# ChaoqinRobotics/LINS---LiDAR-inertial-SLAM

Hardware: NVIDIA H100
Metric: ESKF iterations/sec (higher is better)
Workload: dtype f64 (f32 association)

## Files before the change

lins---lidar-inertial-slam_b200/csrc/cuda/lins_assoc.cuh:

```cuda
#pragma once
#include "lins_assoc_az.cuh"

namespace lins_dev {

constexpr int kGroupLanes = 4;
constexpr int kThreadScanBins = 16, kThreadWalkBins = 48;

constexpr int kCertSlots = 40, kPassSlots = 48;
__device__ __forceinline__ void count_cert_events(long long* timers, unsigned ev) {
#pragma unroll
  for (int k = 0; k < 8; ++k) {
    const unsigned n1 = __popc(__ballot_sync(0xffffffffu, (ev >> k) & 1u)), n2 = __popc(__ballot_sync(0xffffffffu, (ev >> (8 + k)) & 1u));
    if ((threadIdx.x & 31) == 0 && (n1 | n2)) atomicAdd((unsigned long long*)&timers[kCertSlots + k], ((unsigned long long)n2 << 32) | n1);
  }
}

struct PassBuffers {
  float4* qpt;
  float4* sel;
  unsigned long long* key;
  int* pos;
  float4* qa;
  int4* qw;
  float4* qref;
// ... 88 lines not shown
    float4 qa = make_float4(0.f, 0.f, -1.f, 0.f);
    if (seeded) {
      const float4 r1 = pb.qref[v], r2 = pb.qref2[v], ex = pb.qext[v];
      const unsigned nearbits = __float_as_uint(nearf);
      const int w1s = pb.pos[3 * v], w2s = pb.pos[3 * v + 1], w3s = pb.pos[3 * v + 2];
      const int r1s = __float_as_int(ex.y), r2s = __float_as_int(ex.z), r3s = __float_as_int(ex.w);
      const int ccr0 = pb.qccr[v];
      const bool walks = ccr0 >= 0;
      auto entry = [&](int slot, bool use) -> float4 {
        return use && slot >= 0 && slot < ixq.T ? ixq.pts[slot] : make_float4(0.f, 0.f, 0.f, 0.f);
      };
      const float4 tw1 = entry(w1s, true), tr1 = entry(r1s, w1s >= 0);
      const float4 tw2 = entry(w2s, walks), tr2 = entry(r2s, walks && w2s >= 0);
      const float4 tw3 = entry(w3s, walks && surf), tr3 = entry(r3s, walks && surf && w3s >= 0);
      const float moved1 = sqrtf(sqdist_f32(s.x, s.y, s.z, r1.x, r1.y, r1.z));
      const int c1 = w1s >= 0 ? cert_check<false>(tw1, tr1, s, r1s, r1.w, moved1, nearbits, 0)
                              : (cert_rejected(r1.w, moved1) ? kCertKeep : kCertFailSlack);
      const bool ok1 = c1 <= kCertSwap;
      ev = 1u | (1u << (ok1 ? 1 : c1)) | (c1 == kCertSwap ? 1u << 7 : 0u);
      if (c1 == kCertSwap) { az_polar(s, qa); pb.qa[v] = qa; pb.qw[v] = make_int4(-4, 0, 0, 0); continue; }
      bool ok2 = false;
      int c2 = kCertKeep, c3 = kCertKeep;
      if (ok1 && walks) {
        const int c0 = ccr0 & 0x00ffffff;
        const float moved2 = sqrtf(sqdist_f32(s.x, s.y, s.z, r2.x, r2.y, r2.z));
        c2 = w2s >= 0 ? cert_check<true>(tw2, tr2, s, r2s, r2.w, moved2, nearbits, c0) : (cert_rejected(r2.w, moved2) ? kCertKeep : kCertFailSlack);
        ok2 = c2 <= kCertSwap;
        if (ok2 && surf) {
          c3 = w3s >= 0 ? cert_check<true>(tw3, tr3, s, r3s, ex.x, moved2, nearbits, c0) : (cert_rejected(ex.x, moved2) ? kCertKeep : kCertFailSlack);
          ok2 = c3 <= kCertSwap;
        }
        ev |= (1u << 8) | (1u << (8 + (ok2 ? 1 : c2 <= kCertSwap ? c3 : c2))) |
              (ok2 && (c2 == kCertSwap || c3 == kCertSwap) ? 1u << 15 : 0u);
      }
      if (ok1 && (ok2 || ccr0 < 0)) { pb.qw[v] = make_int4(-2, (c2 == kCertSwap ? 1 : 0) | (c3 == kCertSwap ? 2 : 0), 0, 0); continue; }
      if (ok1) { az_polar(s, qa); pb.qa[v] = qa; pb.qw[v] = make_int4(-3, 0, 0, 0); continue; }
    }
    const int w1 = az_prepare_nn(ixq, s, nearf, seeded ? pb.pos[3 * v] : -1, (int)pb.qpt[v].w, qa);
    pb.qa[v] = qa;
    pb.qw[v] = make_int4(w1, 0, 0, 0);
    if (sm.first_pass && w1 >= 0 && (w1 & 0xffff) <= kThreadScanBins) pb.wl[NQ - 1 - atomicAdd(&cta.wl_tn[0], 1)] = v;
    else pb.wl[atomicAdd(&cta.wl_n[0], 1)] = v;
    if (bv.timers && w1 >= 0) atomicAdd(&cta.dbg[0], w1 & 0xffff);
    } while (false);
    if (bv.timers) count_cert_events(bv.timers, ev);
  }
  __syncthreads();
  LINS_TICK_PASS(3);

  if (cta.any_indexed) {
    if (bv.timers && threadIdx.x == 0) {
      atomicAdd((unsigned long long*)&bv.timers[10], (unsigned long long)cta.wl_n[0]);
      atomicAdd((unsigned long long*)&bv.timers[12], (unsigned long long)cta.dbg[0]);
    }
    const float gate = sqrtf(nearf);
    auto nn_finish = [&](int v, const AzIndex& ix, const float4 s, const Top3& top, int w1, float Bout) {
      const unsigned long long k1 = top.k1;
      const int p1 = top.p1;
      const float d1 = __uint_as_float((unsigned)(k1 >> 32));
      const bool acc1 = k1 != kKeyMax && p1 >= 0 && (double)d1 < kp.nearest_sq;
      if (bv.timers && !slots[slot_of(v, Q)].first_pass && pb.pos[3 * v] >= 0 && acc1 && (p1 == pb.pos[3 * v] || p1 == __float_as_int(pb.qext[v].y)))
        atomicAdd((unsigned long long*)&bv.timers[kCertSlots + 6], 1ull);
      const float bound1 = w1 < 0 ? -1.f : acc1 ? cert_bound(top.d3, Bout) : rejected_slack((unsigned)(k1 >> 32), Bout, gate);
      pb.qref[v] = make_float4(s.x, s.y, s.z, bound1);
      pb.qext[v].y = __int_as_float(acc1 ? top.p2 : -1);
      pb.pos[3 * v] = acc1 ? p1 : -1;
      pb.qccr[v] = acc1 ? ((slot_ring(ix.pts[p1].w) << 24) | (int)(unsigned)(k1 & 0xffffffffu)) : -1;
    };
    constexpr int G = kGroupLanes;
    const int sub = lane & (G - 1), glead = lane & ~(G - 1);
    const unsigned gmask = G == 32 ? 0xffffffffu : (((1u << G) - 1u) << glead);
    for (;;) {
      int k = 0;
      if (sub == 0) k = atomicAdd(&cta.wl_thead[0], 1);
      k = __shfl_sync(gmask, k, glead);
      if (k >= cta.wl_tn[0]) break;
      const int v = pb.wl[NQ - 1 - k];
      const int sl = slot_of(v, Q), i = v - sl * Q;
      const Smem& sm = slots[sl];
      const AzIndex ix = az_index_of(sm, bv, i < sm.ns);
      const float4 s = pb.sel[v];
      const int w1 = pb.qw[v].x;
      const float4 qag = pb.qa[v];
      const Top3 top = az_scan_nn_group<G>(ix, s, w1, qag.y, qag.w, sub, gmask);
      if (sub == 0) nn_finish(v, ix, s, top, w1, qag.w);
    }
    for (;;) {
      int k = 0;
      if (lane == 0) k = atomicAdd(&cta.wl_head[0], 1);
      k = __shfl_sync(0xffffffffu, k, 0);
      if (k >= cta.wl_n[0]) break;
      const int v = pb.wl[k];
      const int sl = slot_of(v, Q), i = v - sl * Q;
      const Smem& sm = slots[sl];
      int w1 = pb.qw[v].x;
      Top3 top;
      top.init();
      const bool surf = i < sm.ns;
      const AzIndex ix = az_index_of(sm, bv, surf);
      const float4 s = pb.sel[v];
      float4 qa = pb.qa[v];
      if (w1 >= 0) {
        const int wp = sm.first_pass ? az_probe_window(ix, qa, w1) : -1;
        if (wp >= 0) {
          const Top3 pr = az_scan_nn(ix, s, wp, qa.y, sqrtf(widen(kProbeSq)));
          if (pr.p1 >= 0) {
            w1 = az_nn_window(ix, az_seed_bound(ix, s, pr.p1, nearf), qa);
            if (lane == 0) pb.qa[v] = qa;
          }
        }
        top = az_scan_nn(ix, s, w1, qa.y, qa.w);
      }
      if (lane == 0) nn_finish(v, ix, s, top, w1, qa.w);
    }
    __syncthreads();
    if (bv.timers && threadIdx.x == 0 && !cta.pass_first) {
      const int n = cta.wl_n[0] + cta.wl_tn[0], b = n == 0 ? 0 : n <= 16 ? 1 : 2;
      atomicAdd((unsigned long long*)&bv.timers[kPassSlots + b], 1ull);
      atomicAdd((unsigned long long*)&bv.timers[kPassSlots + 3 + b], (unsigned long long)(clock64() - cta.tlast));
    }
    LINS_TICK_PASS(4);
    for (int v = threadIdx.x; v < NQ; v += kThreads) {
      const int sl = slot_of(v, Q), i = v - sl * Q;
      const Smem& sm = slots[sl];
      if (!sm.run || !sm.az_ok || i >= sm.ns + sm.nc || (sm.iter % kp.icp_freq) != 0) continue;
      const int2 lq = *reinterpret_cast<const int2*>(&pb.qw[v]);
      const int lvl = lq.x;
      const bool surf = i < sm.ns;
      auto swap_front = [&](int k, float* runner_up) {
        const int w = pb.pos[3 * v + k], r = __float_as_int(*runner_up);
        pb.pos[3 * v + k] = r;
        *runner_up = __int_as_float(w);
        return az_index_of(sm, bv, surf).pts[r].w;
      };
      if (lvl == -2) {
        if (lq.y) {
          int* const o = surf ? bv.ind_s + 3 * (size_t)(sm.qs0 + i) : bv.ind_c + 2 * (size_t)(sm.qc0 + i - sm.ns);
          if (lq.y & 1) o[1] = slot_index(swap_front(1, &pb.qext[v].z));
          if (lq.y & 2) o[2] = slot_index(swap_front(2, &pb.qext[v].w));
        }
        continue;
      }
      if (lvl == -4) {
        const float tw = swap_front(0, &pb.qext[v].y);
        pb.qccr[v] = (slot_ring(tw) << 24) | slot_index(tw);
      }
      const int ccr = pb.qccr[v];
      if (ccr < 0) {
        pb.pos[3 * v + 1] = -1; pb.pos[3 * v + 2] = -1;
        pb.qw[v] = make_int4(-1, 0, 0, 0);
        if (surf) { int* o = bv.ind_s + 3 * (size_t)(sm.qs0 + i); o[0] = -1; o[1] = -1; o[2] = -1; }
        else { int* o = bv.ind_c + 2 * (size_t)(sm.qc0 + i - sm.ns); o[0] = -1; o[1] = -1; }
        continue;
      }
      int w2 = 0, w3 = 0;
      float B2 = 0.f, B3 = 0.f;
      const bool seeded = !sm.first_pass;
      const int sd2 = seeded ? pb.pos[3 * v + 1] : -1, sd3 = seeded ? pb.pos[3 * v + 2] : -1;
      const int c = ccr & 0x00ffffff, cr = (int)((unsigned)ccr >> 24);
      const AzIndex ix = az_index_of(sm, bv, surf);
      const int p1 = pb.pos[3 * v];
      if (surf) az_prepare_walk<true>(ix, pb.sel[v], pb.qa[v], p1, c, cr, sd2, sd3, min(sm.ns, sm.Ts), nearf, w2, w3, B2, B3);
      else az_prepare_walk<false>(ix, pb.sel[v], pb.qa[v], p1, c, cr, sd2, sd3, min(sm.nc, sm.Tc), nearf, w2, w3, B2, B3);
      pb.qw[v] = make_int4(lvl == -3 ? 2 : 1, w2, w3, ccr);
      reinterpret_cast<float2*>(pb.key)[v] = make_float2(B2, B3);
      if (sm.first_pass && (w2 & 0xffff) <= kThreadWalkBins && (w3 & 0xffff) <= kThreadWalkBins) pb.wl[NQ - 1 - atomicAdd(&cta.wl_tn[1], 1)] = v;
      else pb.wl[atomicAdd(&cta.wl_n[1], 1)] = v;
      if (bv.timers) atomicAdd(&cta.dbg[1], (w2 & 0xffff) + 4 * (w3 & 0xffff));
    }
    __syncthreads();
    if (bv.timers && threadIdx.x == 0) {
      atomicAdd((unsigned long long*)&bv.timers[11], (unsigned long long)cta.wl_n[1]);
      atomicAdd((unsigned long long*)&bv.timers[13], (unsigned long long)cta.dbg[1]);
    }
    auto walk_finish = [&](int v, const Smem& sm, int i, bool surf, const float4 s, int ccr, const WalkOut& wo) {
      float4 ex = pb.qext[v];
      if (bv.timers && pb.qw[v].x == 2) {
        auto held = [](int w, int r, int now) { return w >= 0 ? now == w || now == r : now < 0; };
        if (held(pb.pos[3 * v + 1], __float_as_int(ex.z), wo.pos2) && (!surf || held(pb.pos[3 * v + 2], __float_as_int(ex.w), wo.pos3)))
          atomicAdd((unsigned long long*)&bv.timers[kCertSlots + 6], 1ull << 32);
      }
      pb.pos[3 * v + 1] = wo.pos2; pb.pos[3 * v + 2] = wo.pos3;
      pb.qref2[v] = make_float4(s.x, s.y, s.z, wo.bound2);
      ex.x = wo.bound3; ex.z = __int_as_float(wo.run2); ex.w = __int_as_float(wo.run3);
      pb.qext[v] = ex;
      const int i1 = ccr & 0x00ffffff;
      if (surf) { int* o = bv.ind_s + 3 * (size_t)(sm.qs0 + i); o[0] = i1; o[1] = wo.i2; o[2] = wo.i3; }
      else { int* o = bv.ind_c + 2 * (size_t)(sm.qc0 + i - sm.ns); o[0] = i1; o[1] = wo.i2; }
    };
    for (;;) {
      int k = 0;
      if (sub == 0) k = atomicAdd(&cta.wl_thead[1], 1);
      k = __shfl_sync(gmask, k, glead);
      if (k >= cta.wl_tn[1]) break;
      const int v = pb.wl[NQ - 1 - k];
      const int sl = slot_of(v, Q), i = v - sl * Q;
      const Smem& sm = slots[sl];
      const int4 w = pb.qw[v];
      const bool surf = i < sm.ns;
      const float2 B = reinterpret_cast<const float2*>(pb.key)[v];
      const float4 s = pb.sel[v];
      const AzIndex ix = az_index_of(sm, bv, surf);
      const WalkOut wo = surf ? az_scan_walk_group<true, G>(ix, s, w.w, w.y, w.z, min(sm.ns, sm.Ts), nearf, B.x, B.y, sub, gmask)
                              : az_scan_walk_group<false, G>(ix, s, w.w, w.y, w.z, min(sm.nc, sm.Tc), nearf, B.x, B.y, sub, gmask);
      if (sub == 0) walk_finish(v, sm, i, surf, s, w.w, wo);
    }
    for (;;) {
      int k = 0;
      if (lane == 0) k = atomicAdd(&cta.wl_head[1], 1);
      k = __shfl_sync(0xffffffffu, k, 0);
      if (k >= cta.wl_n[1]) break;
      const int v = pb.wl[k];
      const int sl = slot_of(v, Q), i = v - sl * Q;
      const Smem& sm = slots[sl];
      const int4 w = pb.qw[v];
      const bool surf = i < sm.ns;
      const float2 B = reinterpret_cast<const float2*>(pb.key)[v];
      const int w2 = w.y, w3 = w.z;
      const float4 s = pb.sel[v];
      const AzIndex ix = az_index_of(sm, bv, surf);
      const WalkOut wo = surf ? az_scan_walk<true>(ix, s, w.w, w2, w3, min(sm.ns, sm.Ts), nearf, B.x, B.y)
                              : az_scan_walk<false>(ix, s, w.w, w2, w3, min(sm.nc, sm.Tc), nearf, B.x, B.y);
      if (lane == 0) walk_finish(v, sm, i, surf, s, w.w, wo);
    }
  }
  if (cta.any_legacy) {
    for (int sl = 0; sl < bv.nslots; ++sl) {
      const Smem& sm = slots[sl];
      if (!sm.run || sm.az_ok || (sm.iter % kp.icp_freq) != 0) continue;
      const bool sep = nn_separate(bv, sm.scan);
      const float4* __restrict__ nnS = sep ? bv.nn_s + bv.nn_s_off[sm.scan] : bv.ts + sm.ts0;
      const float4* __restrict__ nnC = sep ? bv.nn_c + bv.nn_c_off[sm.scan] : bv.tc + sm.tc0;
      const int TnS = sep ? bv.nn_s_off[sm.scan + 1] - bv.nn_s_off[sm.scan] : sm.Ts;
      const int TnC = sep ? bv.nn_c_off[sm.scan + 1] - bv.nn_c_off[sm.scan] : sm.Tc;
      if (sm.ns > 0 && TnS > 0) nn_brute(pb.sel + sl * Q, pb.key + sl * Q, sm.ns, nnS, TnS);
      if (sm.nc > 0 && TnC > 0) nn_brute(pb.sel + sl * Q + sm.ns, pb.key + sl * Q + sm.ns, sm.nc, nnC, TnC);
    }
    __syncthreads();
    for (int sl = 0; sl < bv.nslots; ++sl) {
      const Smem& sm = slots[sl];
      if (!sm.run || sm.az_ok || (sm.iter % kp.icp_freq) != 0) continue;
      const float4* __restrict__ tgtS = bv.ts + sm.ts0;
      const float4* __restrict__ tgtC = bv.tc + sm.tc0;
      const int fwdS = min(sm.ns, sm.Ts), fwdC = min(sm.nc, sm.Tc);
      for (int i = threadIdx.x; i < sm.ns + sm.nc; i += kThreads) {
        const int v = sl * Q + i;
        const bool surf = i < sm.ns;
        const unsigned long long k1 = pb.key[v];
        const float d1 = __uint_as_float((unsigned)(k1 >> 32));
        const int c = (int)(unsigned)(k1 & 0xffffffffu);
        const bool found = (k1 != kKeyMax) && ((double)d1 < kp.nearest_sq) && c < (surf ? sm.Ts : sm.Tc);
        int i1 = -1, i2 = -1, i3 = -1;
        if (found) {
          i1 = c;
          const float4 s = pb.sel[v];
          if (surf) walk_seq<true>(s, c, tgtS, sm.Ts, fwdS, nearf, i2, i3);
          else walk_seq<false>(s, c, tgtC, sm.Tc, fwdC, nearf, i2, i3);
        }
        pb.pos[3 * v] = i1; pb.pos[3 * v + 1] = i2; pb.pos[3 * v + 2] = i3;
        if (surf) { int* o = bv.ind_s + 3 * (size_t)(sm.qs0 + i); o[0] = i1; o[1] = i2; o[2] = i3; }
        else { int* o = bv.ind_c + 2 * (size_t)(sm.qc0 + i - sm.ns); o[0] = i1; o[1] = i2; }
      }
    }
  }
  __syncthreads();
  if (bv.timers && threadIdx.x == 0 && !cta.pass_first) {
    const int n = cta.wl_n[1] + cta.wl_tn[1], b = n == 0 ? 0 : n <= 16 ? 1 : n <= 32 ? 2 : 3;
    atomicAdd((unsigned long long*)&bv.timers[kPassSlots + 6 + b], 1ull);
    atomicAdd((unsigned long long*)&bv.timers[kPassSlots + 10 + b], (unsigned long long)(clock64() - cta.tlast));
  }
  LINS_TICK_PASS(5);
  if (threadIdx.x == kThreads - 1) { cta.wl_n[0] = 0; cta.wl_n[1] = 0; cta.wl_tn[0] = 0; cta.wl_tn[1] = 0; cta.wl_head[0] = 0; cta.wl_head[1] = 0; cta.wl_thead[0] = 0; cta.wl_thead[1] = 0; cta.dbg[0] = 0; cta.dbg[1] = 0; }

  double* const fold_stage = cta.u.fold[warp];
  for (int v0 = warp * 32; v0 < NQ; v0 += kThreads) {
    const int sl = slot_of(v0, Q), i0 = v0 - sl * Q;
    const Smem& sm = slots[sl];
    const int ntot = sm.ns + sm.nc;
    if (!sm.run || i0 >= ntot) continue;
    const int v = v0 + lane, i = i0 + lane;
    const bool valid = i < ntot;
    const bool surf = i < sm.ns;
    const bool search = (sm.iter % kp.icp_freq) == 0;
    const bool weighted = sm.iter >= kp.icp_freq;
    const bool by_slot = search ? (sm.az_ok != 0) : (sm.pos_valid && sm.pos_is_slot);
    float4 coeff = make_float4(0.f, 0.f, 0.f, 0.f);
    float4 s = make_float4(0.f, 0.f, 0.f, 0.f);
    bool ok = false;
    if (valid) {
      const int i1 = pb.pos[3 * v], i2 = pb.pos[3 * v + 1], i3 = pb.pos[3 * v + 2];
      s = pb.sel[v];
      if (surf) {
        if (i2 >= 0 && i3 >= 0 && i1 >= 0 && i1 < sm.Ts && i2 < sm.Ts && i3 < sm.Ts) {
          const float4* t = by_slot ? bv.az_s + sm.ts0 : bv.ts + sm.ts0;
          ok = plane_residual(s, t[i1], t[i2], t[i3], weighted, coeff);
        }
      } else {
        if (i2 >= 0 && i1 >= 0 && i1 < sm.Tc && i2 < sm.Tc) {
          const float4* t = by_slot ? bv.az_c + sm.tc0 : bv.tc + sm.tc0;
          ok = line_residual(s, t[i1], t[i2], weighted, coeff);
        }
      }
    }
    double g[6] = {0.0, 0.0, 0.0, 0.0, 0.0, 0.0}, r = 0.0;
    if (ok) {
// ... 28 lines not shown
```

lins---lidar-inertial-slam_b200/csrc/cuda/lins_assoc_az.cuh:

```cuda
#pragma once
#include "lins_kernels.cuh"

namespace lins_dev {

struct AzIndex {
  const float4* pts;
  const aztab_t* bstart;
  const int (*elev)[2];
  int nb, nrings, T;
};
__device__ __forceinline__ int float_key(float f) { const int i = __float_as_int(f); return i >= 0 ? i : i ^ 0x7fffffff; }
__device__ __forceinline__ float key_float(int k) { return __int_as_float(k >= 0 ? k : k ^ 0x7fffffff); }
__device__ __forceinline__ float slope_of(float x, float y, float z) {
  return __fdiv_rn(z, sqrtf(__fadd_rn(__fmul_rn(x, x), __fmul_rn(y, y))));
}
__device__ __forceinline__ float ring_lower_bound(const AzIndex& ix, int r, float zq, float rq) {
  const float lo = key_float(ix.elev[r][0]), hi = key_float(ix.elev[r][1]);
  const float a = __fmaf_rn(lo, rq, -zq), b = __fmaf_rn(-hi, rq, zq);
  const float m = a > b ? lo : hi;
  const float bound = fmaxf(a, b) * rsqrtf(__fmaf_rn(m, m, 1.f)) * 0.998f - 1.0e-4f;
  return hi - lo < 1.0e30f ? bound : -1.f;
}

__device__ __forceinline__ int az_bin(float x, float y, int nb) {
  const float a = atan2f(y, x);
  int b = (int)floorf((a + kPiF) * ((float)nb * (0.5f / kPiF)));
  return min(max(b, 0), nb - 1);
}
__device__ __forceinline__ int az_bins_for(int nrings, int tab) {
  int p2 = 1;
  while (p2 < nrings) p2 <<= 1;
  return tab / p2;
}

__device__ __forceinline__ int cnt16_add1(unsigned* cnt, int b) {
  const int sh = (b & 1) * 16;
  return (int)((atomicAdd(&cnt[b >> 1], 1u << sh) >> sh) & 0xffffu);
}
template <int TAB>
__device__ void az_build(const float4* __restrict__ src, int T, float4* dst, aztab_t* table, unsigned* cnt, int* scan_tmp, int nb, int (*elev)[2]) {
  unsigned short* cnt16 = reinterpret_cast<unsigned short*>(cnt);
  for (int w = threadIdx.x; w <= TAB / 2; w += kThreads) cnt[w] = 0u;
  for (int r = threadIdx.x; r < kMaxRing; r += kThreads) { elev[r][0] = float_key(3.0e38f); elev[r][1] = float_key(-3.0e38f); }
  __syncthreads();
  for (int j = threadIdx.x; j < T; j += kThreads) {
    const float4 t = __ldg(&src[j]);
    cnt16_add1(cnt, (int)t.w * nb + az_bin(t.x, t.y, nb));
    const float e = slope_of(t.x, t.y, t.z);
    if (fabsf(e) < 1.0e30f) { const int k = float_key(e); atomicMin(&elev[(int)t.w][0], k); atomicMax(&elev[(int)t.w][1], k); }
    else { atomicMin(&elev[(int)t.w][0], float_key(-3.0e38f)); atomicMax(&elev[(int)t.w][1], float_key(3.0e38f)); }
  }
  __syncthreads();
  constexpr int PER = TAB / kThreads;
  static_assert(PER >= 1 && PER * kThreads == TAB, "table size must be a multiple of the block size");
  int loc[PER];
  int sum = 0;
#pragma unroll
  for (int k = 0; k < PER; ++k) { loc[k] = cnt16[threadIdx.x * PER + k]; sum += loc[k]; }
  scan_tmp[threadIdx.x] = sum;
  __syncthreads();
  if (threadIdx.x < 32) {
    constexpr int PW = kThreads / 32;
    int part[PW];
    int s = 0;
#pragma unroll
    for (int k = 0; k < PW; ++k) { part[k] = scan_tmp[threadIdx.x * PW + k]; s += part[k]; }
    int incl = s;
#pragma unroll
    for (int m = 1; m < 32; m <<= 1) { const int o = __shfl_up_sync(0xffffffffu, incl, m); if ((int)threadIdx.x >= m) incl += o; }
    int run = incl - s;
#pragma unroll
    for (int k = 0; k < PW; ++k) { const int v = part[k]; scan_tmp[threadIdx.x * PW + k] = run; run += v; }
    if (threadIdx.x == 31) table[TAB] = (aztab_t)incl;
  }
  __syncthreads();
  {
    int run = scan_tmp[threadIdx.x];
#pragma unroll
    for (int k = 0; k < PER; ++k) { cnt16[threadIdx.x * PER + k] = (unsigned short)run; table[threadIdx.x * PER + k] = (aztab_t)run; run += loc[k]; }
  }
  __syncthreads();
  for (int j = threadIdx.x; j < T; j += kThreads) {
    const float4 t = __ldg(&src[j]);
    const int pos = cnt16_add1(cnt, (int)t.w * nb + az_bin(t.x, t.y, nb));
    dst[pos] = make_float4(t.x, t.y, t.z, __int_as_float(((int)t.w << 24) | j));
  }
  __syncthreads();
}

__device__ __forceinline__ float az_halfwidth(float U, float rho) {
  const float r = sqrtf(U) * 1.002f + 1.0e-5f;
  if (!(r < rho)) return 4.0f;
  return asinf(r / rho) + 1.0e-5f;
}
__device__ __forceinline__ void az_window(int nb, float aq, float th, int& blo, int& nbins) {
  const float inv_binw = (float)nb * (0.5f / kPiF);
  nbins = (int)(2.0f * th * inv_binw) + 3;
  if (!(th < kPiF) || nbins >= nb) { blo = 0; nbins = nb; return; }
  int b = (int)floorf((aq - th + kPiF) * inv_binw) - 1;
  b %= nb;
  if (b < 0) b += nb;
  blo = b;
}

__device__ __forceinline__ int slot_index(float w) { return __float_as_int(w) & 0x00ffffff; }
__device__ __forceinline__ int slot_ring(float w) { return (int)((unsigned)__float_as_int(w) >> 24); }
__device__ __forceinline__ int pack_window(int blo, int nbins) { return (blo << 16) | nbins; }
constexpr float kCertMargin = 0.1f;
__device__ __forceinline__ float widen(float U) { const float r = sqrtf(U) + kCertMargin; return r * r; }
__device__ __forceinline__ float rejected_slack(unsigned best_bits, float Bout, float gate) {
  const float db = best_bits >= 0x7f800000u ? Bout : fminf(sqrtf(__uint_as_float(best_bits)), Bout);
  return db - gate * 1.00001f;
}

__device__ __forceinline__ void az_polar(const float4 s, float4& qa) {
  qa.x = atan2f(s.y, s.x);
  qa.y = sqrtf(__fadd_rn(__fmul_rn(s.x, s.x), __fmul_rn(s.y, s.y)));
}
__device__ __forceinline__ int az_nn_window(const AzIndex& ix, float U1, float4& qa) {
  const float Uw = widen(U1);
  int blo, nbins;
  az_window(ix.nb, qa.x, az_halfwidth(Uw, qa.y), blo, nbins);
  qa.w = nbins >= ix.nb ? 3.0e38f : sqrtf(Uw);
  return pack_window(blo, nbins);
}
__device__ __forceinline__ float az_seed_bound(const AzIndex& ix, const float4 s, int seed_slot, float U1) {
  if (seed_slot >= 0 && seed_slot < ix.T) {
    const float4 t = ix.pts[seed_slot];
    const float d = sqdist_f32(s.x, s.y, s.z, t.x, t.y, t.z);
    if (d < U1) U1 = d;
  }
  return U1;
}
__device__ __forceinline__ int az_bin_of_angle(float a, int nb) {
  const int b = (int)floorf((a + kPiF) * ((float)nb * (0.5f / kPiF)));
  return min(max(b, 0), nb - 1);
}
__device__ __forceinline__ float az_bucket_bound(const AzIndex& ix, const float4 s, float az, int ring_guess, float U1) {
  const int bq = az_bin_of_angle(az, ix.nb);
  const int r0 = min(max(ring_guess, 0), ix.nrings - 1);
#pragma unroll 1
  for (int k = 0; k < 3; ++k) {
    const int r = k == 0 ? r0 : (k == 1 ? r0 - 1 : r0 + 1);
    if (k == 1 && U1 < 1.0f) break;
    if (r < 0 || r >= ix.nrings) continue;
    const int base = r * ix.nb;
    int p = ix.bstart[base + max(bq - 1, 0)];
    const int pe = min((int)ix.bstart[base + min(bq + 2, ix.nb)], p + 4);
    for (; p < pe; ++p) U1 = az_seed_bound(ix, s, p, U1);
  }
  return U1;
}
__device__ __forceinline__ int az_prepare_nn(const AzIndex& ix, const float4 s, float nearf, int seed_slot, int ring_guess, float4& qa) {
  qa = make_float4(0.f, 0.f, -1.f, 0.f);
  if (!(s.x == s.x && s.y == s.y && s.z == s.z) || ix.T <= 0) return -1;
  az_polar(s, qa);
  float U1 = az_seed_bound(ix, s, seed_slot, nearf);
  if (seed_slot < 0) U1 = az_bucket_bound(ix, s, qa.x, ring_guess, U1);
  return az_nn_window(ix, U1, qa);
}
constexpr float kProbeSq = 0.25f;
__device__ __forceinline__ int az_probe_window(const AzIndex& ix, const float4 qa, int full_window) {
  int blo, nbins;
  az_window(ix.nb, qa.x, az_halfwidth(kProbeSq, qa.y), blo, nbins);
  return (full_window & 0xffff) > 2 * nbins + 4 ? pack_window(blo, nbins) : -1;
}

struct Top3 {
  unsigned long long k1, k2;
  int p1, p2;
  unsigned d3;
  __device__ __forceinline__ void init() { k1 = kKeyMax; k2 = kKeyMax; p1 = -1; p2 = -1; d3 = 0xffffffffu; }
  __device__ __forceinline__ void insert(unsigned long long k, int p) {
    const bool lt1 = k < k1, lt2 = k < k2;
    d3 = lt2 ? (unsigned)(k2 >> 32) : min(d3, (unsigned)(k >> 32));
    k2 = lt1 ? k1 : (lt2 ? k : k2);
    p2 = lt1 ? p1 : (lt2 ? p : p2);
    k1 = lt1 ? k : k1;
    p1 = lt1 ? p : p1;
  }
};
__device__ __forceinline__ int warp_argmin_lane(unsigned long long k, unsigned long long& kmin) {
  const unsigned hi = (unsigned)(k >> 32), lo = (unsigned)(k & 0xffffffffu);
  const unsigned mhi = __reduce_min_sync(0xffffffffu, hi);
  const unsigned mlo = __reduce_min_sync(0xffffffffu, hi == mhi ? lo : 0xffffffffu);
  kmin = ((unsigned long long)mhi << 32) | mlo;
  return __ffs(__ballot_sync(0xffffffffu, hi == mhi && lo == mlo)) - 1;
}
__device__ __forceinline__ void warp_top3(Top3& t) {
  const int lane = threadIdx.x & 31;
  unsigned long long K1, K2;
  const int a = warp_argmin_lane(t.k1, K1);
  const int P1 = __shfl_sync(0xffffffffu, t.p1, a);
  const unsigned long long cand = lane == a ? t.k2 : t.k1;
  const int candp = lane == a ? t.p2 : t.p1;
  const int b = warp_argmin_lane(cand, K2);
  const int P2 = __shfl_sync(0xffffffffu, candp, b);
  unsigned rest;
  if (lane == a && lane == b) rest = t.d3;
  else if (lane == a || lane == b) rest = (unsigned)(t.k2 >> 32);
  else rest = (unsigned)(t.k1 >> 32);
  t.d3 = __reduce_min_sync(0xffffffffu, rest);
  t.k1 = K1; t.p1 = K1 == kKeyMax ? -1 : P1;
  t.k2 = K2; t.p2 = K2 == kKeyMax ? -1 : P2;
}
__device__ __forceinline__ float cert_bound(unsigned third_bits, float Bout) {
  return third_bits >= 0x7f800000u ? Bout : fminf(sqrtf(__uint_as_float(third_bits)), Bout);
}
__device__ __forceinline__ float4 ld_slot(const AzIndex& ix, int p) { return ix.pts[p]; }
template <int LPR>
__device__ __forceinline__ void az_scan_nn_slice(const AzIndex& ix, const float4 s, int p, int pe, Top3& top) {
  for (; p < pe; p += 4 * LPR) {
    unsigned long long k[4];
    int q[4];
    float4 tt[4];
#pragma unroll
    for (int u = 0; u < 4; ++u) tt[u] = ld_slot(ix, p + u * LPR < pe ? p + u * LPR : p);
#pragma unroll
    for (int u = 0; u < 4; ++u) {
      const int pu = p + u * LPR;
      const bool valid = pu < pe;
      const float4 t = tt[u];
      const unsigned d = __float_as_uint(sqdist_f32(s.x, s.y, s.z, t.x, t.y, t.z));
      k[u] = valid ? (((unsigned long long)d << 32) | (unsigned)slot_index(t.w)) : kKeyMax;
      q[u] = pu;
    }
#pragma unroll
    for (int u = 0; u < 4; ++u) top.insert(k[u], q[u]);
  }
}
template <int LPR>
__device__ __forceinline__ Top3 az_scan_nn_t(const AzIndex& ix, const float4 s, int win, float rq, float Bout, long long* tm = nullptr) {
  const int lane = threadIdx.x & 31;
  const int blo = win >> 16, nbins = win & 0xffff;
  constexpr int RPP = 32 / LPR;
  const int sub = lane % LPR;
  Top3 top;
  top.init();
  const int e0 = min(blo + nbins, ix.nb), e1 = blo + nbins - ix.nb;
  int dbg_cand = 0;
  for (int rbase = 0; rbase < ix.nrings; rbase += RPP) {
    const int r = rbase + lane / LPR;
    if (r < ix.nrings && !(ring_lower_bound(ix, r, s.z, rq) > Bout)) {
      const int base = r * ix.nb;
      if (tm) { dbg_cand += max(0, (ix.bstart[base + e0] - ix.bstart[base + blo] - sub + LPR - 1) / LPR); if (e1 > 0) dbg_cand += max(0, (ix.bstart[base + e1] - ix.bstart[base] - sub + LPR - 1) / LPR); }
      az_scan_nn_slice<LPR>(ix, s, ix.bstart[base + blo] + sub, ix.bstart[base + e0], top);
      if (e1 > 0) az_scan_nn_slice<LPR>(ix, s, ix.bstart[base] + sub, ix.bstart[base + e1], top);
    }
  }
  if (tm) { tm[0] = clock64(); tm[2] = __reduce_max_sync(0xffffffffu, (unsigned)dbg_cand); tm[3] = __reduce_add_sync(0xffffffffu, (unsigned)dbg_cand); }
  warp_top3(top);
  if ((unsigned)(top.k1 >> 32) >= 0x7f800000u) { top.k1 = kKeyMax; top.p1 = -1; }
  if (tm) tm[1] = clock64();
  return top;
}
__device__ __forceinline__ Top3 az_scan_nn(const AzIndex& ix, const float4 s, int win, float rq, float Bout, long long* tm = nullptr) {
  if (ix.nrings <= 8) return az_scan_nn_t<4>(ix, s, win, rq, Bout, tm);
  if (ix.nrings <= 16) return az_scan_nn_t<2>(ix, s, win, rq, Bout, tm);
  return az_scan_nn_t<1>(ix, s, win, rq, Bout, tm);
}

template <int G>
__device__ __forceinline__ void group_top3(Top3& t, unsigned gmask) {
#pragma unroll
  for (int m = 1; m < G; m <<= 1) {
    const unsigned long long ok1 = __shfl_xor_sync(gmask, t.k1, m), ok2 = __shfl_xor_sync(gmask, t.k2, m);
    const int op1 = __shfl_xor_sync(gmask, t.p1, m), op2 = __shfl_xor_sync(gmask, t.p2, m);
    const unsigned od3 = __shfl_xor_sync(gmask, t.d3, m);
    t.insert(ok1, op1);
    t.insert(ok2, op2);
    t.d3 = min(t.d3, od3);
  }
}
__device__ __forceinline__ void az_scan_slice_lane(const AzIndex& ix, const float4 s, int p, int pe, int step, Top3& top) {
  for (; p < pe; p += 2 * step) {
    const int p1 = p + step;
    const float4 t0 = ld_slot(ix, p), t1 = ld_slot(ix, p1 < pe ? p1 : p);
    const unsigned d0 = __float_as_uint(sqdist_f32(s.x, s.y, s.z, t0.x, t0.y, t0.z));
    const unsigned d1 = __float_as_uint(sqdist_f32(s.x, s.y, s.z, t1.x, t1.y, t1.z));
    top.insert(((unsigned long long)d0 << 32) | (unsigned)slot_index(t0.w), p);
    top.insert(p1 < pe ? (((unsigned long long)d1 << 32) | (unsigned)slot_index(t1.w)) : kKeyMax, p1);
  }
}
template <int G>
__device__ __forceinline__ Top3 az_scan_nn_group(const AzIndex& ix, const float4 s, int win, float rq, float Bout, int sub, unsigned gmask) {
  const int blo = win >> 16, nbins = win & 0xffff;
  const int e0 = min(blo + nbins, ix.nb), e1 = blo + nbins - ix.nb;
  Top3 top;
  top.init();
  for (int r = sub; r < ix.nrings; r += G) {
    if (ring_lower_bound(ix, r, s.z, rq) > Bout) continue;
    const int base = r * ix.nb;
    az_scan_slice_lane(ix, s, ix.bstart[base + blo], ix.bstart[base + e0], 1, top);
    if (e1 > 0) az_scan_slice_lane(ix, s, ix.bstart[base], ix.bstart[base + e1], 1, top);
  }
  group_top3<G>(top, gmask);
  if ((unsigned)(top.k1 >> 32) >= 0x7f800000u) { top.k1 = kKeyMax; top.p1 = -1; }
  return top;
}

template <bool SURF, bool CLS2>
__device__ __forceinline__ float seed_bound(const float4 t, bool valid, const float4 s, int c, int cr, int fwdBound, float U) {
  const int j = slot_index(t.w), r = slot_ring(t.w);
  const bool ring_ok = (SURF && CLS2) ? (r == cr) : (r != cr && r >= cr - 2 && r <= cr + 2);
  const float d = sqdist_f32(t.x, t.y, t.z, s.x, s.y, s.z);
  return (valid && ring_ok && j != c && (j < c || j < fwdBound) && d < U) ? d : U;
}
template <bool SURF>
__device__ __forceinline__ void az_prepare_walk(const AzIndex& ix, const float4 s, const float4 qa, int p1, int c, int cr, int seed2,
                                                int seed3, int fwdBound, float Uinit, int& w2, int& w3, float& B2, float& B3) {
  auto fetch = [&](int seed, bool& valid) -> float4 {
    valid = seed >= 0 && seed < ix.T;
    return valid ? ix.pts[seed] : make_float4(0.f, 0.f, 0.f, 0.f);
  };
  float U2 = Uinit, U3 = Uinit;
  {
    constexpr int NA = SURF ? 6 : 1;
    const int seeds[6] = {seed2, seed3, p1 - 2, p1 - 1, p1 + 1, p1 + 2};
    float4 t[NA];
    bool ok[NA];
#pragma unroll
    for (int k = 0; k < NA; ++k) t[k] = fetch(seeds[k], ok[k]);
    U2 = seed_bound<SURF, true>(t[0], ok[0], s, c, cr, fwdBound, U2);
    if (SURF) {
      U3 = seed_bound<SURF, false>(t[1 % NA], ok[1 % NA], s, c, cr, fwdBound, U3);
#pragma unroll
      for (int k = 2; k < NA; ++k) U2 = seed_bound<true, true>(t[k], ok[k], s, c, cr, fwdBound, U2);
    }
  }
  {
    const int bq = az_bin_of_angle(qa.x, ix.nb);
    float& U = SURF ? U3 : U2;
    float4 t[8];
    bool ok[8];
#pragma unroll
    for (int k = 0; k < 4; ++k) {
      const int r = cr + (k < 2 ? k - 2 : k - 1);
      const bool rok = r >= 0 && r < ix.nrings;
      const int slot = rok ? (int)ix.bstart[r * ix.nb + bq] : -1;
      t[2 * k] = fetch(slot, ok[2 * k]);
      t[2 * k + 1] = fetch(rok ? slot - 1 : -1, ok[2 * k + 1]);
    }
#pragma unroll
    for (int k = 0; k < 8; ++k) U = seed_bound<SURF, !SURF>(t[k], ok[k], s, c, cr, fwdBound, U);
  }
  int blo, nbins;
  const float Uw2 = widen(U2);
  az_window(ix.nb, qa.x, az_halfwidth(Uw2, qa.y), blo, nbins);
  w2 = pack_window(blo, nbins);
  B2 = nbins >= ix.nb ? 3.0e38f : sqrtf(Uw2);
  if (SURF) {
    const float Uw3 = widen(U3);
    az_window(ix.nb, qa.x, az_halfwidth(Uw3, qa.y), blo, nbins);
    w3 = pack_window(blo, nbins);
    B3 = nbins >= ix.nb ? 3.0e38f : sqrtf(Uw3);
  } else { w3 = w2; B3 = B2; }
}

constexpr int kWalkInFlight = 4;
constexpr int kGroupWalkInFlight = 4;
struct WalkOut {
  int i2, i3, pos2, pos3, run2, run3;
  float bound2, bound3;
};
template <bool SURF>
__device__ __forceinline__ WalkOut az_scan_walk(const AzIndex& ix, const float4 s, int ccr, int w2, int w3, int fwdBound, float nearf,
                                                float B2, float B3) {
  const int lane = threadIdx.x & 31;
  const int c = ccr & 0x00ffffff, cr = (int)((unsigned)ccr >> 24);
  Top3 top;
  top.init();
  constexpr int LPR = SURF ? 7 : 8;
  const int q = lane / LPR;
  const bool own = SURF && q >= 4;
  const int r = own ? cr : cr + (q < 2 ? q - 2 : q - 1);
  const int sub = own ? lane - 4 * LPR : lane - q * LPR, step = own ? 4 : LPR;
  const bool cls2 = SURF ? own : true;
  if (r >= 0 && r < ix.nrings) {
    const int win = cls2 ? w2 : w3;
    const int blo = win >> 16, nbins = win & 0xffff, base = r * ix.nb;
    for (int seg = 0; seg < 2; ++seg) {
      int p, pe;
      if (seg == 0) { p = ix.bstart[base + blo]; pe = ix.bstart[base + min(blo + nbins, ix.nb)]; }
      else { const int e1 = blo + nbins - ix.nb; if (e1 <= 0) break; p = ix.bstart[base]; pe = ix.bstart[base + e1]; }
      for (p += sub; p < pe; p += kWalkInFlight * step) {
        float4 tt[kWalkInFlight];
#pragma unroll
        for (int u = 0; u < kWalkInFlight; ++u) tt[u] = ld_slot(ix, p + step * u < pe ? p + step * u : p);
#pragma unroll
        for (int u = 0; u < kWalkInFlight; ++u) {
          const int pu = p + step * u;
          const float4 t = tt[u];
          const unsigned d = __float_as_uint(sqdist_f32(t.x, t.y, t.z, s.x, s.y, s.z));
          const int j = slot_index(t.w);
          const bool fwd = j > c;
          const bool adm = pu < pe && j != c && (!fwd || j < fwdBound);
          const unsigned long long k = adm ? (((unsigned long long)d << 32) | (fwd ? order_fwd(j) : order_bwd(j))) : kKeyMax;
          top.insert(k, pu);
        }
      }
    }
  }
  const float gate = sqrtf(nearf);
  const unsigned nearbits = __float_as_uint(nearf);
  const bool mine2 = cls2;
  Top3 neutral;
  neutral.init();
  WalkOut o;
  auto finish = [&](Top3 t, float Bout, int& idx, int& pos, int& run, float& bound) {
    warp_top3(t);
    const bool ok = (unsigned)(t.k1 >> 32) < nearbits && t.p1 >= 0;
    idx = ok ? order_decode((unsigned)(t.k1 & 0xffffffffu)) : -1;
    pos = ok ? t.p1 : -1;
    run = ok ? t.p2 : -1;
    bound = ok ? cert_bound(t.d3, Bout) : rejected_slack((unsigned)(t.k1 >> 32), Bout, gate);
  };
  finish(mine2 ? top : neutral, B2, o.i2, o.pos2, o.run2, o.bound2);
  if (SURF) finish(mine2 ? neutral : top, B3, o.i3, o.pos3, o.run3, o.bound3);
  else { o.i3 = -1; o.pos3 = -1; o.run3 = -1; o.bound3 = 0.f; }
  return o;
}

template <bool SURF, int G>
__device__ __forceinline__ WalkOut az_scan_walk_group(const AzIndex& ix, const float4 s, int ccr, int w2, int w3, int fwdBound, float nearf,
                                                      float B2, float B3, int sub, unsigned gmask) {
  const int c = ccr & 0x00ffffff, cr = (int)((unsigned)ccr >> 24);
  Top3 t2, t3;
  t2.init(); t3.init();
  auto scan_ring = [&](int r, int win, Top3& top, int start, int step) {
    const int blo = win >> 16, nbins = win & 0xffff, base = r * ix.nb;
    for (int seg = 0; seg < 2; ++seg) {
      int p, pe;
      if (seg == 0) { p = ix.bstart[base + blo]; pe = ix.bstart[base + min(blo + nbins, ix.nb)]; }
      else { const int e1 = blo + nbins - ix.nb; if (e1 <= 0) break; p = ix.bstart[base]; pe = ix.bstart[base + e1]; }
      for (p += start; p < pe; p += kGroupWalkInFlight * step) {
        float4 tt[kGroupWalkInFlight];
#pragma unroll
        for (int u = 0; u < kGroupWalkInFlight; ++u) tt[u] = ld_slot(ix, p + u * step < pe ? p + u * step : p);
#pragma unroll
        for (int u = 0; u < kGroupWalkInFlight; ++u) {
          const int pu = p + u * step;
          const float4 t = tt[u];
          const unsigned d = __float_as_uint(sqdist_f32(t.x, t.y, t.z, s.x, s.y, s.z));
          const int j = slot_index(t.w);
          const bool fwd = j > c;
          const bool adm = pu < pe && j != c && (!fwd || j < fwdBound);
          top.insert(adm ? (((unsigned long long)d << 32) | (fwd ? order_fwd(j) : order_bwd(j))) : kKeyMax, pu);
        }
      }
    }
  };
  if (SURF && cr < ix.nrings) scan_ring(cr, w2, t2, sub, G);
  for (int idx = sub; idx < 4; idx += G) {
    const int r = cr + (idx < 2 ? idx - 2 : idx - 1);
    if (r < 0 || r >= ix.nrings) continue;
    if (SURF) scan_ring(r, w3, t3, 0, 1); else scan_ring(r, w2, t2, 0, 1);
  }
  group_top3<G>(t2, gmask);
  if (SURF) group_top3<G>(t3, gmask);
  const float gate = sqrtf(nearf);
  const unsigned nearbits = __float_as_uint(nearf);
  WalkOut o;
  auto finish = [&](const Top3& t, float Bout, int& idx, int& pos, int& run, float& bound) {
    const bool ok = (unsigned)(t.k1 >> 32) < nearbits && t.p1 >= 0;
    idx = ok ? order_decode((unsigned)(t.k1 & 0xffffffffu)) : -1;
    pos = ok ? t.p1 : -1;
    run = ok ? t.p2 : -1;
    bound = ok ? cert_bound(t.d3, Bout) : rejected_slack((unsigned)(t.k1 >> 32), Bout, gate);
  };
  finish(t2, B2, o.i2, o.pos2, o.run2, o.bound2);
  if (SURF) finish(t3, B3, o.i3, o.pos3, o.run3, o.bound3);
  else { o.i3 = -1; o.pos3 = -1; o.run3 = -1; o.bound3 = 0.f; }
  return o;
}

enum : int { kCertKeep = 0, kCertSwap = 1, kCertFailRunnerUp = 2, kCertFailBound = 3, kCertFailGate = 4, kCertFailSlack = 5 };
template <bool WALK>
__device__ __forceinline__ int cert_check(const float4 tw, const float4 tr, const float4 s, int r, float bound, float moved, unsigned nearbits,
                                          int c) {
  auto key_of = [&](const float4 t) -> unsigned long long {
    const unsigned d = __float_as_uint(sqdist_f32(t.x, t.y, t.z, s.x, s.y, s.z));
    const int j = slot_index(t.w);
    const unsigned lo = WALK ? (j > c ? order_fwd(j) : order_bwd(j)) : (unsigned)j;
    return ((unsigned long long)d << 32) | lo;
  };
  const unsigned long long kw = key_of(tw), kr = r >= 0 ? key_of(tr) : kKeyMax;
  const bool swap = kr < kw;
  const unsigned dm = (unsigned)((swap ? kr : kw) >> 32);
  if (!(dm < nearbits)) return kCertFailGate;
  if (!(sqrtf(__uint_as_float(dm)) + moved + 2.0e-4f < bound)) return swap ? kCertFailRunnerUp : kCertFailBound;
  return swap ? kCertSwap : kCertKeep;
}
__device__ __forceinline__ bool cert_rejected(float slack, float moved) { return slack > 0.f && 2.0f * moved + 2.0e-4f < slack; }

}
```

Baseline: 7.260 million.

## Tighten certification bounds using exact azimuth-window geometry and skipped-ring bounds

Replaces the conservative certificate bound (sqrt of the widened search radius) with a geometric bound computed from the actual azimuth window: the chord distance to the window edge at the query's range, via a sine polynomial. The NN scans also return the minimum lower bound over rings they skipped, and this tightens the first-neighbour bound. The precomputed B2/B3 values stored in pb.key are dropped and recomputed from qa in the walk finish. Tighter bounds should let more later iterations certify cached neighbours and skip rescans, at the cost of extra arithmetic and a reduction, plus some risk to correctness if the bound is not conservative.

```diff
diff --git a/lins---lidar-inertial-slam_b200/csrc/cuda/lins_assoc.cuh b/lins---lidar-inertial-slam_b200/csrc/cuda/lins_assoc.cuh
--- a/lins---lidar-inertial-slam_b200/csrc/cuda/lins_assoc.cuh
+++ b/lins---lidar-inertial-slam_b200/csrc/cuda/lins_assoc.cuh
@@ -194,8 +194,9 @@
       const float4 s = pb.sel[v];
       const int w1 = pb.qw[v].x;
       const float4 qag = pb.qa[v];
-      const Top3 top = az_scan_nn_group<G>(ix, s, w1, qag.y, qag.w, sub, gmask);
-      if (sub == 0) nn_finish(v, ix, s, top, w1, qag.w);
+      float Bout = 3.0e38f;
+      const Top3 top = az_scan_nn_group<G>(ix, s, w1, qag.y, qag.w, Bout, sub, gmask);
+      if (sub == 0) nn_finish(v, ix, s, top, w1, Bout);
     }
     for (;;) {
       int k = 0;
@@ -212,18 +213,19 @@
       const AzIndex ix = az_index_of(sm, bv, surf);
       const float4 s = pb.sel[v];
       float4 qa = pb.qa[v];
+      float Bout = 3.0e38f;
       if (w1 >= 0) {
         const int wp = sm.first_pass ? az_probe_window(ix, qa, w1) : -1;
         if (wp >= 0) {
-          const Top3 pr = az_scan_nn(ix, s, wp, qa.y, sqrtf(widen(kProbeSq)));
+          const Top3 pr = az_scan_nn(ix, s, wp, qa.y, sqrtf(widen(kProbeSq)), Bout);
           if (pr.p1 >= 0) {
             w1 = az_nn_window(ix, az_seed_bound(ix, s, pr.p1, nearf), qa);
-            if (lane == 0) pb.qa[v] = qa;
+            if (lane == 0) { pb.qa[v] = qa; pb.qw[v].x = w1; }
           }
         }
-        top = az_scan_nn(ix, s, w1, qa.y, qa.w);
-      }
-      if (lane == 0) nn_finish(v, ix, s, top, w1, qa.w);
+        top = az_scan_nn(ix, s, w1, qa.y, qa.w, Bout);
+      }
+      if (lane == 0) nn_finish(v, ix, s, top, w1, Bout);
     }
     __syncthreads();
     if (bv.timers && threadIdx.x == 0 && !cta.pass_first) {
@@ -239,6 +241,12 @@
       const int2 lq = *reinterpret_cast<const int2*>(&pb.qw[v]);
       const int lvl = lq.x;
       const bool surf = i < sm.ns;
+      if (lvl >= 0) {
+        const float4 qa = pb.qa[v];
+        const float Bwin = az_outside_bound(surf ? sm.nbS : sm.nbC, lvl, qa.x, qa.y);
+        float* const b1 = &pb.qref[v].w;
+        *b1 = fminf(*b1, pb.qccr[v] >= 0 ? Bwin : rejected_slack(0xffffffffu, Bwin, gate));
+      }
       auto swap_front = [&](int k, float* runner_up) {
         const int w = pb.pos[3 * v + k], r = __float_as_int(*runner_up);
         pb.pos[3 * v + k] = r;
@@ -266,16 +274,14 @@
         continue;
       }
       int w2 = 0, w3 = 0;
-      float B2 = 0.f, B3 = 0.f;
       const bool seeded = !sm.first_pass;
       const int sd2 = seeded ? pb.pos[3 * v + 1] : -1, sd3 = seeded ? pb.pos[3 * v + 2] : -1;
       const int c = ccr & 0x00ffffff, cr = (int)((unsigned)ccr >> 24);
       const AzIndex ix = az_index_of(sm, bv, surf);
       const int p1 = pb.pos[3 * v];
-      if (surf) az_prepare_walk<true>(ix, pb.sel[v], pb.qa[v], p1, c, cr, sd2, sd3, min(sm.ns, sm.Ts), nearf, w2, w3, B2, B3);
-      else az_prepare_walk<false>(ix, pb.sel[v], pb.qa[v], p1, c, cr, sd2, sd3, min(sm.nc, sm.Tc), nearf, w2, w3, B2, B3);
+      if (surf) az_prepare_walk<true>(ix, pb.sel[v], pb.qa[v], p1, c, cr, sd2, sd3, min(sm.ns, sm.Ts), nearf, w2, w3);
+      else az_prepare_walk<false>(ix, pb.sel[v], pb.qa[v], p1, c, cr, sd2, sd3, min(sm.nc, sm.Tc), nearf, w2, w3);
       pb.qw[v] = make_int4(lvl == -3 ? 2 : 1, w2, w3, ccr);
-      reinterpret_cast<float2*>(pb.key)[v] = make_float2(B2, B3);
       if (sm.first_pass && (w2 & 0xffff) <= kThreadWalkBins && (w3 & 0xffff) <= kThreadWalkBins) pb.wl[NQ - 1 - atomicAdd(&cta.wl_tn[1], 1)] = v;
       else pb.wl[atomicAdd(&cta.wl_n[1], 1)] = v;
       if (bv.timers) atomicAdd(&cta.dbg[1], (w2 & 0xffff) + 4 * (w3 & 0xffff));
@@ -310,11 +316,11 @@
       const Smem& sm = slots[sl];
       const int4 w = pb.qw[v];
       const bool surf = i < sm.ns;
-      const float2 B = reinterpret_cast<const float2*>(pb.key)[v];
+      const float4 qa = pb.qa[v];
       const float4 s = pb.sel[v];
       const AzIndex ix = az_index_of(sm, bv, surf);
-      const WalkOut wo = surf ? az_scan_walk_group<true, G>(ix, s, w.w, w.y, w.z, min(sm.ns, sm.Ts), nearf, B.x, B.y, sub, gmask)
-                              : az_scan_walk_group<false, G>(ix, s, w.w, w.y, w.z, min(sm.nc, sm.Tc), nearf, B.x, B.y, sub, gmask);
+      const WalkOut wo = surf ? az_scan_walk_group<true, G>(ix, s, w.w, w.y, w.z, min(sm.ns, sm.Ts), nearf, qa, sub, gmask)
+                              : az_scan_walk_group<false, G>(ix, s, w.w, w.y, w.z, min(sm.nc, sm.Tc), nearf, qa, sub, gmask);
       if (sub == 0) walk_finish(v, sm, i, surf, s, w.w, wo);
     }
     for (;;) {
@@ -327,12 +333,12 @@
       const Smem& sm = slots[sl];
       const int4 w = pb.qw[v];
       const bool surf = i < sm.ns;
-      const float2 B = reinterpret_cast<const float2*>(pb.key)[v];
+      const float4 qa = pb.qa[v];
       const int w2 = w.y, w3 = w.z;
       const float4 s = pb.sel[v];
       const AzIndex ix = az_index_of(sm, bv, surf);
-      const WalkOut wo = surf ? az_scan_walk<true>(ix, s, w.w, w2, w3, min(sm.ns, sm.Ts), nearf, B.x, B.y)
-                              : az_scan_walk<false>(ix, s, w.w, w2, w3, min(sm.nc, sm.Tc), nearf, B.x, B.y);
+      const WalkOut wo = surf ? az_scan_walk<true>(ix, s, w.w, w2, w3, min(sm.ns, sm.Ts), nearf, qa)
+                              : az_scan_walk<false>(ix, s, w.w, w2, w3, min(sm.nc, sm.Tc), nearf, qa);
       if (lane == 0) walk_finish(v, sm, i, surf, s, w.w, wo);
     }
   }
diff --git a/lins---lidar-inertial-slam_b200/csrc/cuda/lins_assoc_az.cuh b/lins---lidar-inertial-slam_b200/csrc/cuda/lins_assoc_az.cuh
--- a/lins---lidar-inertial-slam_b200/csrc/cuda/lins_assoc_az.cuh
+++ b/lins---lidar-inertial-slam_b200/csrc/cuda/lins_assoc_az.cuh
@@ -101,6 +101,16 @@
   b %= nb;
   if (b < 0) b += nb;
   blo = b;
+}
+
+__device__ __forceinline__ float az_outside_bound(int nb, int win, float aq, float rho) {
+  const int blo = win >> 16, nbins = win & 0xffff;
+  if (nbins >= nb) return 3.0e38f;
+  float u = (aq + kPiF) * ((float)nb * (0.5f / kPiF)) - (float)blo;
+  if (u < 0.f) u += (float)nb;
+  const float D = fminf(fmaxf(fminf(u, (float)nbins - u) * (2.0f * kPiF / (float)nb) - 1.0e-5f, 0.f), 0.5f * kPiF);
+  const float D2 = D * D;
+  return rho * (D * (1.0f - D2 * (1.0f / 6.0f - D2 * (1.0f / 120.0f - D2 * (1.0f / 5040.0f))))) / 1.002f - 1.0e-5f;
 }
 
 __device__ __forceinline__ int slot_index(float w) { return __float_as_int(w) & 0x00ffffff; }
@@ -230,7 +240,7 @@
   }
 }
 template <int LPR>
-__device__ __forceinline__ Top3 az_scan_nn_t(const AzIndex& ix, const float4 s, int win, float rq, float Bout, long long* tm = nullptr) {
+__device__ __forceinline__ Top3 az_scan_nn_t(const AzIndex& ix, const float4 s, int win, float rq, float Bout, float& Bcert, long long* tm = nullptr) {
   const int lane = threadIdx.x & 31;
   const int blo = win >> 16, nbins = win & 0xffff;
   constexpr int RPP = 32 / LPR;
@@ -239,9 +249,12 @@
   top.init();
   const int e0 = min(blo + nbins, ix.nb), e1 = blo + nbins - ix.nb;
   int dbg_cand = 0;
+  float skip = Bcert;
   for (int rbase = 0; rbase < ix.nrings; rbase += RPP) {
     const int r = rbase + lane / LPR;
-    if (r < ix.nrings && !(ring_lower_bound(ix, r, s.z, rq) > Bout)) {
+    const float lb = r < ix.nrings ? ring_lower_bound(ix, r, s.z, rq) : -1.f;
+    if (lb > Bout) skip = fminf(skip, lb);
+    else if (r < ix.nrings) {
       const int base = r * ix.nb;
       if (tm) { dbg_cand += max(0, (ix.bstart[base + e0] - ix.bstart[base + blo] - sub + LPR - 1) / LPR); if (e1 > 0) dbg_cand += max(0, (ix.bstart[base + e1] - ix.bstart[base] - sub + LPR - 1) / LPR); }
       az_scan_nn_slice<LPR>(ix, s, ix.bstart[base + blo] + sub, ix.bstart[base + e0], top);
@@ -249,15 +262,16 @@
     }
   }
   if (tm) { tm[0] = clock64(); tm[2] = __reduce_max_sync(0xffffffffu, (unsigned)dbg_cand); tm[3] = __reduce_add_sync(0xffffffffu, (unsigned)dbg_cand); }
+  Bcert = key_float((int)__reduce_min_sync(0xffffffffu, (unsigned)(float_key(skip) ^ 0x80000000)) ^ 0x80000000);
   warp_top3(top);
   if ((unsigned)(top.k1 >> 32) >= 0x7f800000u) { top.k1 = kKeyMax; top.p1 = -1; }
   if (tm) tm[1] = clock64();
   return top;
 }
-__device__ __forceinline__ Top3 az_scan_nn(const AzIndex& ix, const float4 s, int win, float rq, float Bout, long long* tm = nullptr) {
-  if (ix.nrings <= 8) return az_scan_nn_t<4>(ix, s, win, rq, Bout, tm);
-  if (ix.nrings <= 16) return az_scan_nn_t<2>(ix, s, win, rq, Bout, tm);
-  return az_scan_nn_t<1>(ix, s, win, rq, Bout, tm);
+__device__ __forceinline__ Top3 az_scan_nn(const AzIndex& ix, const float4 s, int win, float rq, float Bout, float& Bcert, long long* tm = nullptr) {
+  if (ix.nrings <= 8) return az_scan_nn_t<4>(ix, s, win, rq, Bout, Bcert, tm);
+  if (ix.nrings <= 16) return az_scan_nn_t<2>(ix, s, win, rq, Bout, Bcert, tm);
+  return az_scan_nn_t<1>(ix, s, win, rq, Bout, Bcert, tm);
 }
 
 template <int G>
@@ -283,17 +297,23 @@
   }
 }
 template <int G>
-__device__ __forceinline__ Top3 az_scan_nn_group(const AzIndex& ix, const float4 s, int win, float rq, float Bout, int sub, unsigned gmask) {
+__device__ __forceinline__ Top3 az_scan_nn_group(const AzIndex& ix, const float4 s, int win, float rq, float Bout, float& Bcert, int sub,
+                                                 unsigned gmask) {
   const int blo = win >> 16, nbins = win & 0xffff;
   const int e0 = min(blo + nbins, ix.nb), e1 = blo + nbins - ix.nb;
   Top3 top;
   top.init();
+  float skip = Bcert;
   for (int r = sub; r < ix.nrings; r += G) {
-    if (ring_lower_bound(ix, r, s.z, rq) > Bout) continue;
+    const float lb = ring_lower_bound(ix, r, s.z, rq);
+    if (lb > Bout) { skip = fminf(skip, lb); continue; }
     const int base = r * ix.nb;
     az_scan_slice_lane(ix, s, ix.bstart[base + blo], ix.bstart[base + e0], 1, top);
     if (e1 > 0) az_scan_slice_lane(ix, s, ix.bstart[base], ix.bstart[base + e1], 1, top);
   }
+#pragma unroll
+  for (int m = 1; m < G; m <<= 1) skip = fminf(skip, __shfl_xor_sync(gmask, skip, m));
+  Bcert = skip;
   group_top3<G>(top, gmask);
   if ((unsigned)(top.k1 >> 32) >= 0x7f800000u) { top.k1 = kKeyMax; top.p1 = -1; }
   return top;
@@ -308,7 +328,7 @@
 }
 template <bool SURF>
 __device__ __forceinline__ void az_prepare_walk(const AzIndex& ix, const float4 s, const float4 qa, int p1, int c, int cr, int seed2,
-                                                int seed3, int fwdBound, float Uinit, int& w2, int& w3, float& B2, float& B3) {
+                                                int seed3, int fwdBound, float Uinit, int& w2, int& w3) {
   auto fetch = [&](int seed, bool& valid) -> float4 {
     valid = seed >= 0 && seed < ix.T;
     return valid ? ix.pts[seed] : make_float4(0.f, 0.f, 0.f, 0.f);
@@ -345,16 +365,12 @@
     for (int k = 0; k < 8; ++k) U = seed_bound<SURF, !SURF>(t[k], ok[k], s, c, cr, fwdBound, U);
   }
   int blo, nbins;
-  const float Uw2 = widen(U2);
-  az_window(ix.nb, qa.x, az_halfwidth(Uw2, qa.y), blo, nbins);
+  az_window(ix.nb, qa.x, az_halfwidth(widen(U2), qa.y), blo, nbins);
   w2 = pack_window(blo, nbins);
-  B2 = nbins >= ix.nb ? 3.0e38f : sqrtf(Uw2);
   if (SURF) {
-    const float Uw3 = widen(U3);
-    az_window(ix.nb, qa.x, az_halfwidth(Uw3, qa.y), blo, nbins);
+    az_window(ix.nb, qa.x, az_halfwidth(widen(U3), qa.y), blo, nbins);
     w3 = pack_window(blo, nbins);
-    B3 = nbins >= ix.nb ? 3.0e38f : sqrtf(Uw3);
-  } else { w3 = w2; B3 = B2; }
+  } else w3 = w2;
 }
 
 constexpr int kWalkInFlight = 4;
@@ -365,7 +381,7 @@
 };
 template <bool SURF>
 __device__ __forceinline__ WalkOut az_scan_walk(const AzIndex& ix, const float4 s, int ccr, int w2, int w3, int fwdBound, float nearf,
-                                                float B2, float B3) {
+                                                const float4 qa) {
   const int lane = threadIdx.x & 31;
   const int c = ccr & 0x00ffffff, cr = (int)((unsigned)ccr >> 24);
   Top3 top;
@@ -407,23 +423,24 @@
   Top3 neutral;
   neutral.init();
   WalkOut o;
-  auto finish = [&](Top3 t, float Bout, int& idx, int& pos, int& run, float& bound) {
+  auto finish = [&](Top3 t, int win, int& idx, int& pos, int& run, float& bound) {
     warp_top3(t);
     const bool ok = (unsigned)(t.k1 >> 32) < nearbits && t.p1 >= 0;
     idx = ok ? order_decode((unsigned)(t.k1 & 0xffffffffu)) : -1;
     pos = ok ? t.p1 : -1;
     run = ok ? t.p2 : -1;
+    const float Bout = az_outside_bound(ix.nb, win, qa.x, qa.y);
     bound = ok ? cert_bound(t.d3, Bout) : rejected_slack((unsigned)(t.k1 >> 32), Bout, gate);
   };
-  finish(mine2 ? top : neutral, B2, o.i2, o.pos2, o.run2, o.bound2);
-  if (SURF) finish(mine2 ? neutral : top, B3, o.i3, o.pos3, o.run3, o.bound3);
+  finish(mine2 ? top : neutral, w2, o.i2, o.pos2, o.run2, o.bound2);
+  if (SURF) finish(mine2 ? neutral : top, w3, o.i3, o.pos3, o.run3, o.bound3);
   else { o.i3 = -1; o.pos3 = -1; o.run3 = -1; o.bound3 = 0.f; }
   return o;
 }
 
 template <bool SURF, int G>
 __device__ __forceinline__ WalkOut az_scan_walk_group(const AzIndex& ix, const float4 s, int ccr, int w2, int w3, int fwdBound, float nearf,
-                                                      float B2, float B3, int sub, unsigned gmask) {
+                                                      const float4 qa, int sub, unsigned gmask) {
   const int c = ccr & 0x00ffffff, cr = (int)((unsigned)ccr >> 24);
   Top3 t2, t3;
   t2.init(); t3.init();
@@ -461,15 +478,16 @@
   const float gate = sqrtf(nearf);
   const unsigned nearbits = __float_as_uint(nearf);
   WalkOut o;
-  auto finish = [&](const Top3& t, float Bout, int& idx, int& pos, int& run, float& bound) {
+  auto finish = [&](const Top3& t, int win, int& idx, int& pos, int& run, float& bound) {
     const bool ok = (unsigned)(t.k1 >> 32) < nearbits && t.p1 >= 0;
     idx = ok ? order_decode((unsigned)(t.k1 & 0xffffffffu)) : -1;
     pos = ok ? t.p1 : -1;
     run = ok ? t.p2 : -1;
+    const float Bout = az_outside_bound(ix.nb, win, qa.x, qa.y);
     bound = ok ? cert_bound(t.d3, Bout) : rejected_slack((unsigned)(t.k1 >> 32), Bout, gate);
   };
-  finish(t2, B2, o.i2, o.pos2, o.run2, o.bound2);
-  if (SURF) finish(t3, B3, o.i3, o.pos3, o.run3, o.bound3);
+  finish(t2, w2, o.i2, o.pos2, o.run2, o.bound2);
+  if (SURF) finish(t3, w3, o.i3, o.pos3, o.run3, o.bound3);
   else { o.i3 = -1; o.pos3 = -1; o.run3 = -1; o.bound3 = 0.f; }
   return o;
 }
```

Result: no change. 7.306 million (median of 6 runs) (+0.6%).
